# rrahn/libspm

Measured on AMD Instinct MI355X. Metric: Gbases/s scanned, Myers k<=3 |P|=100, higher is better.
Workload: dtype u32

## Files before the change

### libspm_amd/csrc/filter_dense.hpp

```cpp
#pragma once

#include "filter_stream.hpp"

namespace spm_hip
{

constexpr uint32_t kDenseQueueCap = 192;
constexpr int kDenseBatches = 3;

template <int NP>
__device__ __forceinline__ uint32_t dense_select(const filter_params &P, uint32_t w, uint32_t prev)
{
    const uint32_t X = alignbit(w, prev, 2);
    const uint32_t Y = alignbit(w, prev, 4);
    uint32_t sel = 0;
#pragma unroll
    for (int i = 0; i < NP; ++i) {
        const uint32_t C0 = (P.pat_c[i] & 3u) * 0x55555555u, M0 = (P.pat_cm[i] & 3u) * 0x55555555u;
        const uint32_t C1 = (P.pat_c[i] >> 2) * 0x55555555u, M1 = (P.pat_cm[i] >> 2) * 0x55555555u;
        uint32_t t = ((X ^ C0) & M0) | ((Y ^ C1) & M1);
        t |= t >> 1;
        sel |= ~t;
    }
    return sel & 0x55555555u;
// ... 38 lines not shown
            const uint32_t x0 = bk[b].x ^ f2, x1 = bk[b].y ^ f2, x2 = bk[b].z ^ f2, x3 = bk[b].w ^ f2;
            const uint32_t z = ((x0 - 0x00010001u) & ~x0) | ((x1 - 0x00010001u) & ~x1) | ((x2 - 0x00010001u) & ~x2) |
                               ((x3 - 0x00010001u) & ~x3);
            const bool hit = v[b] && ((z & 0x80008000u) != 0 || (bk[b].w >> 16) == kDenseAcceptAll);
            if (__ballot(hit) != 0) {
                if (__builtin_amdgcn_readfirstlane(cand_chunk_of(P, lds)[5]) == 0) {
                    const int64_t ts = (int64_t)span_base + (int64_t)off[b] - 16;
                    const bool has = hit && ts >= (int64_t)P.lo && (uint64_t)ts + P.key_len <= P.hi;
                    emit_survivors(P, has, key[b], has ? (uint64_t)ts : 0, lane, lds);
                }
            }
        }
    }
}

template <int UU, int NP, int S, bool KM>
__device__ __forceinline__ void dense_group(const filter_params &P, const uint4 (&cur)[UU], uint64_t gbase, uint64_t span_base,
                                            uint32_t &carry_in, uint32_t lane, const uint32_t *lds, dense_queue &Q, uint32_t &qn)
{
    static_assert(UU % 2 == 0 || UU == 1, "words are taken in pairs");
    uint32_t w[UU], prev[UU];
#pragma unroll
    for (int u = 0; u < UU; ++u)
        pack_with_prev(cur[u], lane, carry_in, w[u], prev[u]);
    const uint32_t goff = (uint32_t)(gbase - span_base) + lane * 16;
#pragma unroll
    for (int j = 0; j < UU; j += 2) {
        constexpr bool pair = UU > 1;
        const uint32_t w0 = w[j], p0 = prev[j], w1 = w[pair ? j + 1 : j], p1 = prev[pair ? j + 1 : j];
        const uint32_t kmask = KM ? P.key_mask : 0xFFFFFFFFu;
        static_assert(kDenseBloomBits == 20, "the word address below takes bits 5..19 of the index");
        uint32_t pm = 0;
        if constexpr (S == 0) {
            uint32_t todo = dense_select<NP>(P, w0, p0);
            if (pair)
                todo |= dense_select<NP>(P, w1, p1) << 1;
            while (todo != 0) {
                const uint32_t b = (uint32_t)__ffs(todo) - 1u;
                todo &= todo - 1;
                const bool odd = (b & 1u) != 0;
                const uint64_t both = ((uint64_t)(odd ? w1 : w0) << 32) | (odd ? p1 : p0);
                const uint32_t key = (uint32_t)(both >> ((b & ~1u) + 2u));
                const uint32_t h = key ^ (key >> 13);
                const uint32_t word = *reinterpret_cast<const uint32_t *>(reinterpret_cast<const uint8_t *>(lds) + ((h >> 3) & 0x1FFFCu));
                pm |= __builtin_amdgcn_ubfe(word, h, 1) << b;
            }
        } else {
#pragma unroll
            for (int u = 0; u < (pair ? 2 : 1); ++u) {
#pragma unroll
                for (int d = S; d <= 16; d += S) {
                    const uint32_t wu = u ? w1 : w0, pu = u ? p1 : p0;
                    const uint32_t key = (d == 16 ? wu : alignbit(wu, pu, (2 * d) & 31)) & kmask;
                    const uint32_t h = key ^ (key >> 13);
                    const uint32_t word = *reinterpret_cast<const uint32_t *>(reinterpret_cast<const uint8_t *>(lds) + ((h >> 3) & 0x1FFFCu));
                    pm |= __builtin_amdgcn_ubfe(word, h, 1) << (2 * (d - 1) + u);
                }
            }
        }
        while (__ballot(pm != 0) != 0) {
            const bool pos = pm != 0;
            const uint32_t b = pos ? (uint32_t)__ffs(pm) - 1u : 0u;
            pm &= pm - 1;
            const bool odd = (b & 1u) != 0;
            const uint64_t both = ((uint64_t)(odd ? w1 : w0) << 32) | (odd ? p1 : p0);
            const uint32_t key = (uint32_t)(both >> ((b & ~1u) + 2u)) & kmask;
            const uint64_t mm = __ballot(pos);
            if (pos) {
                const uint32_t q = qn + __popcll(mm & ((1ull << lane) - 1));
                Q.key[q] = key;
                Q.off[q] = goff + (uint32_t)j * 1024u + (odd ? 1024u : 0u) + (b >> 1) + 1u;
            }
            qn += __popcll(mm);
            queue_sync();
            if (qn > kDenseQueueCap - 64)
                dense_drain(P, Q, qn, false, span_base, lane, lds);
        }
    }
}

template <int U, int NP, int S = 0, bool KM = false>
__global__ __launch_bounds__(1024) void seed_filter_dense_kernel(const filter_params P)
{
    extern __shared__ uint32_t lds[];
    stream_stage(P, lds);

    const uint32_t lane = threadIdx.x & 63;
    const uint32_t waves_per_wg = blockDim.x >> 6;
    const uint32_t wave_in_wg = (uint32_t)__builtin_amdgcn_readfirstlane(threadIdx.x >> 6);
    dense_queue &Q = *reinterpret_cast<dense_queue *>(lds + P.lds_words + kCandLdsSlot + kCandRec * 16 +
                                                      (sizeof(dense_queue) / 4) * wave_in_wg);
    uint32_t qn = 0;

    const stream_geometry G = stream_geometry_of(P.lo, P.hi, 1024, P.span_chunks);
    const uint64_t span = P.span_chunks;
    const uint8_t *lane_text = P.text + G.base0 + (uint64_t)lane * 16;

    uint64_t sp;
    for (;;) {
        const span_draw drawn = draw_span(P, lds, lane, wave_in_wg, waves_per_wg, G.n_spans, sp);
        if (drawn == span_draw::done)
            break;
        if (drawn == span_draw::idle)
            continue;
        const uint64_t c_begin = sp * span;
        const uint64_t c_end = c_begin + span < G.n_chunks ? c_begin + span : G.n_chunks;
        const uint64_t span_base = G.base0 + c_begin * 1024;
        span_open(P, lds, lane, span_base);
        uint32_t carry_in = span_carry_in(P, span_base, lane);
        uint64_t ch = c_begin;
        const uint64_t whole_end = c_end < G.n_whole ? c_end : G.n_whole;
        const uint64_t fast_end = c_begin + (whole_end > c_begin ? (whole_end - c_begin) / U * U : 0);
        if (ch < fast_end) {
            uint4 nxt[U];
#pragma unroll
            for (int u = 0; u < U; ++u)
                nxt[u] = load16_stream(lane_text + (ch + u) * 1024);
            for (; ch < fast_end; ch += U) {
                uint4 cur[U];
#pragma unroll
                for (int u = 0; u < U; ++u)
                    cur[u] = nxt[u];
                const bool more = ch + U < fast_end;
                const uint64_t pf = more ? ch + U : ch;
                const uint64_t ustride = more ? 1024 : 0;
#pragma unroll
                for (int u = 0; u < U; ++u)
                    nxt[u] = load16_stream(lane_text + pf * 1024 + (uint64_t)u * ustride);
                __builtin_amdgcn_sched_barrier(0);
                dense_group<U, NP, S, KM>(P, cur, G.base0 + ch * 1024, span_base, carry_in, lane, lds, Q, qn);
            }
        }
        for (; ch < c_end; ++ch) {
            uint4 one[1];
            one[0] = load_text16(P.text, G.base0 + ch * 1024 + (uint64_t)lane * 16, P.hi);
            dense_group<1, NP, S, KM>(P, one, G.base0 + ch * 1024, span_base, carry_in, lane, lds, Q, qn);
        }
        dense_drain(P, Q, qn, true, span_base, lane, lds);
    }
    surv_close(P, cand_chunk_of(P, lds), lane);
}

}
```

### libspm_amd/csrc/filter_resolve.hpp

```cpp
#pragma once

#include "filter_params.hpp"
#include "pack.hpp"
#include "wave.hpp"

namespace spm_hip
{


__device__ __forceinline__ uint4 load_bytes16(const uint8_t *p)
{
    uint4 v;
    __builtin_memcpy(&v, p, 16);
    return v;
}

__device__ __forceinline__ uint4 load_bytes16_guarded(const uint8_t *base, uint64_t idx, uint64_t limit)
{
    if (idx + 16 <= limit)
        return load_bytes16(base + idx);
    uint32_t w[4] = {0xFFFFFFFFu, 0xFFFFFFFFu, 0xFFFFFFFFu, 0xFFFFFFFFu};
    for (int b = 0; b < 16; ++b)
        if (idx + b < limit)
            w[b >> 2] = (w[b >> 2] & ~(0xFFu << (8 * (b & 3)))) | ((uint32_t)base[idx + b] << (8 * (b & 3)));
// ... 306 lines not shown
        return;
    }
    if (live && through) {
        ++S.n_cand;
        d_hi = (int64_t)t - (int64_t)(val & 0x7FF) - sb + (int64_t)R.max_m;
        d_lo = d_hi - (int64_t)((rng & kRngRun) ? (rng & 0x7FF) : 0u);
        b_cur = d_lo / (int64_t)R.Bw;
        b_last = d_hi / (int64_t)R.Bw;
        if (R.overlap && b_cur > 0 && d_lo - b_cur * (int64_t)R.Bw <= (int64_t)R.k[pat])
            --b_cur;
        if ((uint64_t)b_last >> R.band_bits) {
            atomicAdd(&R.counters[kCntVoid], 1ull);
            b_last = b_cur - 1;
        }
    }
    for (;;) {
        const bool have = b_cur <= b_last;
        const uint64_t mm = __ballot(have);
        if (mm == 0)
            break;
        if (have) {
            const unsigned long long bkey =
                ((unsigned long long)pat << 43) | ((unsigned long long)seg << R.band_bits) | (unsigned long long)b_cur;
            const int64_t b0 = b_cur * (int64_t)R.Bw;
            const uint32_t o_lo = (uint32_t)(d_lo > b0 ? d_lo - b0 : 0);
            const uint32_t o_hi = (uint32_t)(d_hi < b0 + (int64_t)R.Bw - 1 ? d_hi - b0 : (int64_t)R.Bw - 1);
            const unsigned long long run = (o_hi - o_lo >= 63 ? ~0ull : ((1ull << (o_hi - o_lo + 1)) - 1)) << o_lo;
            const uint32_t q = S.bn + __popcll(mm & ((1ull << lane) - 1));
            B.key_lo[q] = (uint32_t)bkey;
            B.key_hi[q] = (uint32_t)(bkey >> 32);
            B.run_lo[q] = (uint32_t)run;
            B.run_hi[q] = (uint32_t)(run >> 32);
        }
        S.bn += __popcll(mm);
        queue_sync();
        if (S.bn >= 64) {
            S.bn -= 64;
            insert_bands(R, B, S.bn, 64, lane, S.C);
            queue_sync();
        }
        ++b_cur;
    }
    queue_sync();
}

__global__ __launch_bounds__(256) void resolve_kernel(const resolve_params R)
{
    __shared__ pair_queue pair_queues[4];
    __shared__ band_queue band_queues[4];
    unsigned long long n = R.counters[kCntSurvSlots];
    if (blockIdx.x == 0 && threadIdx.x == 0) {
        atomicAdd(&R.counters[kCntUnreadSurvSum], n);
        atomicMax(&R.counters[kCntUnreadSurvMax], n);
    }
    if (n > R.surv_cap)
        n = R.surv_cap;
    if (!R.exact_hits && __hip_atomic_load(R.table_poison, __ATOMIC_RELAXED, __HIP_MEMORY_SCOPE_AGENT) != 0) {
        if (blockIdx.x == 0 && threadIdx.x == 0)
            atomicAdd(&R.counters[kCntVoid], 1ull);
        return;
    }
    const uint32_t lane = threadIdx.x & 63;
    resolve_wave S;
    S.Q = &pair_queues[threadIdx.x >> 6];
    S.B = &band_queues[threadIdx.x >> 6];
    S.qn = 0;
    S.bn = 0;
    S.C.base = 0;
    S.C.used = 0;
    S.C.size = 0;
    S.C.draws = 0;
    S.n_cand = 0;
    pair_queue &Q = *S.Q;
    const uint64_t stride = (uint64_t)gridDim.x * blockDim.x;
    const uint64_t rounds = (n + stride - 1) / stride;
    for (uint64_t r = 0; r < rounds; ++r) {
        if ((r & 7u) == 7u &&
            __builtin_amdgcn_readfirstlane((uint32_t)(__hip_atomic_load(&R.counters[kCntVoid], __ATOMIC_RELAXED, __HIP_MEMORY_SCOPE_AGENT) != 0)))
            break;
        const uint64_t i = r * stride + (uint64_t)blockIdx.x * blockDim.x + threadIdx.x;
        bool probing = false;
        uint32_t key = 0;
        uint64_t t = 0, seg = 0;
        pass_entry T = R.passes[0];
        if (i < n) {
            const survivor sv = R.surv[i];
            if (sv.t_hi != kSurvInvalid) {
                probing = true;
                key = sv.key;
                t = ((uint64_t)sv.t_hi << 32) | sv.t_lo;
                if (sv.pad != 0)
                    T = R.passes[sv.pad];
            }
        }
        if (probing && R.seg_offsets) {
            uint64_t lo = 0, hi = R.n_segments;
            while (hi - lo > 1) {
                const uint64_t mid = (lo + hi) >> 1;
                if (R.seg_offsets[mid] <= t)
                    lo = mid;
                else
                    hi = mid;
            }
            seg = lo;
            if ((int64_t)t + (int64_t)R.key_len > (int64_t)R.seg_offsets[lo + 1])
                probing = false;
        }
        text64 W;
        W.lo = 0;
        W.hi = 0;
        W.ok = false;
        if (probing && R.flank_check) {
            int64_t sb = (int64_t)R.hay_begin, se = (int64_t)R.hay_end;
            if (R.seg_offsets) {
                sb = (int64_t)R.seg_offsets[seg];
                se = (int64_t)R.seg_offsets[seg + 1];
            }
            if ((int64_t)t - 16 >= sb && (int64_t)t + 48 <= se && t + 48 <= R.text_alloc) {
                const uint8_t *p = R.text + (t - 16);
                W.lo = (uint64_t)pack16(load_bytes16(p)) | ((uint64_t)pack16(load_bytes16(p + 16)) << 32);
                W.hi = (uint64_t)pack16(load_bytes16(p + 32)) | ((uint64_t)pack16(load_bytes16(p + 48)) << 32);
                W.ok = true;
            }
        }
        uint32_t first = 0, cnt = 0;
        {
            uint32_t slot = ht_hash(key) & T.ht_mask;
            while (__ballot(probing) != 0) {
                if (probing) {
                    const uint4 d = T.ht[slot];
                    if (d.z == 0) {
                        probing = false;
                    } else if (d.x == key) {
                        first = d.y;
                        cnt = d.z;
                        probing = false;
                    } else {
                        slot = (slot + 1) & T.ht_mask;
                    }
                }
            }
        }
        uint32_t incl = cnt;
#pragma unroll
        for (int o = 1; o < 64; o <<= 1) {
            const uint32_t up = (uint32_t)__shfl_up((int)incl, o);
            if (lane >= (uint32_t)o)
                incl += up;
        }
        const uint32_t total = (uint32_t)__builtin_amdgcn_readfirstlane(__shfl((int)incl, 63));
        for (uint32_t p0 = 0; p0 < total; p0 += 64) {
            const uint32_t i = p0 + lane;
            bool have = i < total;
            uint32_t owner = 0;
#pragma unroll
            for (int step = 32; step > 0; step >>= 1) {
                const uint32_t v = (uint32_t)__shfl((int)incl, (int)(owner + step - 1));
                if (v <= i)
                    owner += step;
            }
            owner = owner > 63 ? 63 : owner;
            const uint32_t o_incl = (uint32_t)__shfl((int)incl, (int)owner), o_cnt = (uint32_t)__shfl((int)cnt, (int)owner);
            const uint32_t o_first = (uint32_t)__shfl((int)first, (int)owner);
            const uint64_t o_t = ((uint64_t)(uint32_t)__shfl((int)(uint32_t)(t >> 32), (int)owner) << 32) |
                                 (uint32_t)__shfl((int)(uint32_t)t, (int)owner);
            const uint32_t o_seg = (uint32_t)__shfl((int)(uint32_t)seg, (int)owner);
            text64 OW;
            OW.lo = ((uint64_t)(uint32_t)__shfl((int)(uint32_t)(W.lo >> 32), (int)owner) << 32) |
                    (uint32_t)__shfl((int)(uint32_t)W.lo, (int)owner);
            OW.hi = ((uint64_t)(uint32_t)__shfl((int)(uint32_t)(W.hi >> 32), (int)owner) << 32) |
                    (uint32_t)__shfl((int)(uint32_t)W.hi, (int)owner);
            OW.ok = __shfl((int)W.ok, (int)owner) != 0;
            uint32_t val = 0, rng = 0;
            if (have) {
                const uint4 e = R.entries[o_first + (i - (o_incl - o_cnt))];
                val = e.x;
                rng = e.z;
                if (!(rng & kRngRun)) {
                    const uint32_t r0 = rng & 0x1F, ns = (rng >> 5) & 0x1F;
                    const bool whole = (rng & kRngWhole) != 0;
                    rng = (r0 << 16) | (whole ? (ns << 5) | kRngWhole : 0u);
                    if (OW.ok) {
                        if (!seed_sig_ok(OW, e.y, r0, ns, R.key_len))
                            have = false;
                        else if (whole)
                            rng |= kSeedChecked;
                    }
                }
            }
            const uint64_t mm = __ballot(have);
            if (mm != 0) {
                if (have) {
                    const uint32_t q = S.qn + __popcll(mm & ((1ull << lane) - 1));
                    Q.t_lo[q] = (uint32_t)o_t;
                    Q.t_hi[q] = (uint32_t)(o_t >> 32);
                    Q.val[q] = val;
                    Q.rng[q] = rng;
                    Q.seg[q] = o_seg;
                }
                S.qn += __popcll(mm);
                queue_sync();
                while (S.qn >= 64)
                    check_pairs(R, S, 64, lane);
            }
        }
    }
    while (S.qn != 0)
        check_pairs(R, S, S.qn < 64 ? S.qn : 64, lane);
    if (S.bn != 0)
        insert_bands(R, *S.B, 0, S.bn, lane, S.C);
    for (uint32_t q = S.C.used + lane; q < S.C.size; q += 64)
        if (S.C.base + q < R.band_cap)
            R.bands[S.C.base + q].val = kBandInvalid;
    wave_count_add(R.counters + kCntPairs, S.n_cand);
}

}
```

### libspm_amd/csrc/filter_stream.hip

```cpp
#include "filter_launch.hpp"
#include "filter_stream.hpp"

namespace
{
using packed_kernel = void (*)(filter_params, const uint4 *);

template <int S, int U, bool KM>
filter_kernel sparse_kernel(uint32_t hv, uint32_t sigma)
{
    if (hv == 2 && sigma == 5)
        return seed_filter_kernel<S, U, 2, 5, KM>;
    if (hv == 2 && sigma == 15)
        return seed_filter_kernel<S, U, 2, 15, KM>;
    if (hv == 1 && sigma == 4)
        return seed_filter_kernel<S, U, 1, 4, KM>;
    if constexpr (S >= 4)
        if (hv == 2 && sigma == 4)
            return seed_filter_kernel<S, U, 2, 4, KM>;
    return nullptr;
}

filter_kernel select_filter_kernel(const filter_index &F, uint32_t sigma, bool km)
{
    if (F.dense || F.hash_variant == 4)
        return select_dense_kernel(F, km);
    switch (F.stride) {
    case 16: return km ? nullptr : sparse_kernel<16, 8, false>(F.hash_variant, sigma);
    case 8: return km ? nullptr : sparse_kernel<8, 8, false>(F.hash_variant, sigma);
    case 4: return km ? nullptr : sparse_kernel<4, 8, false>(F.hash_variant, sigma);
    case 2: return km ? sparse_kernel<2, 2, true>(F.hash_variant, sigma) : sparse_kernel<2, 2, false>(F.hash_variant, sigma);
    case 1:
        if (F.anchor_cm != 0 && F.hash_variant == 2 && sigma == 4 && !km)
            return seed_filter_kernel<1, 4, 2, 4, false, true>;
        return km ? sparse_kernel<1, 2, true>(F.hash_variant, sigma) : sparse_kernel<1, 2, false>(F.hash_variant, sigma);
    default: return nullptr;
    }
}

packed_kernel select_packed_kernel(uint32_t stride, bool km)
{
    if (km)
        return nullptr;
    switch (stride) {
    case 16: return seed_filter_packed_kernel<16, 4, 2, false>;
    case 8: return seed_filter_packed_kernel<8, 4, 2, false>;
    case 4: return seed_filter_packed_kernel<4, 2, 2, false>;
    default: return nullptr;
    }
}

}

int launch_stream_pass(const scan_args &A, filter_params P, uint32_t pass)
{
    spm_ctx *ctx = A.ctx;
    const spm_patterns *ps = A.ps;
    spm_hits *H = A.hits;
    const filter_index &F = ps->fidx[pass];
    P.stride = F.stride;
    P.key_len = F.key_len;
    P.key_mask = F.key_len >= 16 ? 0xFFFFFFFFu : ((1u << (2 * F.key_len)) - 1);
    P.bitmap_words = F.hash_variant == 2 ? 1024 : F.bitmap_words;
    P.lds_words = F.lds_words;
    P.chd_slot_mask = F.chd_slot_mask;
    P.chd_bucket_shift = F.chd_bucket_shift;
    P.chd_disp_off = F.chd_disp_off;
    P.n_probes = F.n_probes;
    P.bitmap = F.d_bitmap;
    P.pass = pass;
    P.anchor_c = F.anchor_c;
    P.anchor_cm = F.anchor_cm;
    P.n_pat = F.n_pat;
    for (uint32_t i = 0; i < kDensePatterns; ++i) {
        P.pat_c[i] = F.pat_c[i];
        P.pat_cm[i] = F.pat_cm[i];
    }
    P.bucket_shift = F.bucket_shift;
    P.buckets = reinterpret_cast<const uint4 *>(F.d_buckets);
    const bool km = F.key_len < 16;
    const bool bits = F.hash_variant == 4;
    const bool use_packed = F.hash_variant == 2 && A.text->d_packed && ps->sigma == 4 && F.stride >= 2 &&
                            !(A.opts.flags & SPM_SCAN_IGNORE_PACKED);
    const bool wide_ok = use_packed || F.stride == 2 || (F.stride == 1 && !km && ps->sigma == 4);
    const uint32_t threads = (F.dense || bits || wide_ok) ? 1024 : 512;
    const size_t lds = (size_t)F.lds_words * 4 + 16 + 16 * kCandRec * 4 + ((F.dense || bits) ? 16 * kDenseQueueBytes : 0);
    const uint32_t wg_per_cu = (uint32_t)std::max<size_t>(1, std::min<size_t>((160 * 1024) / lds, 2048 / threads));
    const uint32_t grid = ctx->n_cu * wg_per_cu;
    const uint64_t n_waves = (uint64_t)grid * (threads / 64);
    const span_plan span = plan_span(stream_geometry_of(P.lo, P.hi, 1024).n_chunks, n_waves, 1024);
    P.span_chunks = span.span_chunks;
    P.span_unit = 1024;
    const int sb = A.tune.span_budget;
    P.span_budget = sb > 0 ? (uint32_t)sb : (uint32_t)std::max<uint64_t>(256, (uint64_t)span.span_chunks * 1024 / 4);
    P.dynamic = span.dynamic;
    P.hash_variant = F.hash_variant;
    H->stats.span_symbols = P.span_chunks * P.span_unit;
    if (use_packed) {
        filter_params Q = P;
        const span_plan pspan = plan_span(stream_geometry_of(Q.lo, Q.hi, 4096).n_chunks, n_waves, 4096);
        Q.span_chunks = pspan.span_chunks;
        Q.span_unit = 4096;
        if (sb <= 0)
            Q.span_budget = (uint32_t)std::max<uint64_t>(256, (uint64_t)pspan.span_chunks * 4096 / 4);
        Q.dynamic = pspan.dynamic;
        H->stats.span_symbols = Q.span_chunks * Q.span_unit;
        const packed_kernel k = select_packed_kernel(F.stride, km);
        if (!k) {
            SPM_SET_ERR(ctx, "internal: no packed filter kernel for stride %u, key length %u", F.stride, F.key_len);
            return SPM_E_UNSUPPORTED;
        }
        launch(k, dim3(grid), threads, lds, ctx->stream, Q, reinterpret_cast<const uint4 *>(A.text->d_packed));
    } else {
        const filter_kernel k = select_filter_kernel(F, ps->sigma, km);
        if (!k) {
            SPM_SET_ERR(ctx, "internal: no filter kernel for stride %u, key length %u, sigma %u, hash variant %u, %u patterns",
                        F.stride, F.key_len, ps->sigma, F.hash_variant, F.n_pat);
            return SPM_E_UNSUPPORTED;
        }
        launch(k, dim3(grid), threads, lds, ctx->stream, P);
    }
    return SPM_OK;
}

void warm_stream_kernels()
{
    hipFuncAttributes a;
    (void)hipFuncGetAttributes(&a, (const void *)seed_filter_kernel<16, 8, 2, 4, false>);
}
```

### libspm_amd/csrc/filter_stream.hpp

```cpp
#pragma once

#include "brute.hpp"
#include "filter_params.hpp"
#include "pack.hpp"

namespace spm_hip
{

__device__ __forceinline__ uint32_t *cand_chunk_of(const filter_params &P, const uint32_t *lds)
{
    const uint32_t wave = (uint32_t)__builtin_amdgcn_readfirstlane(threadIdx.x >> 6);
    return const_cast<uint32_t *>(lds) + P.lds_words + kCandLdsSlot + kCandRec * wave;
}

__device__ __forceinline__ void span_open(const filter_params &P, const uint32_t *lds, uint32_t lane, uint64_t begin)
{
    if (lane == 0) {
        uint32_t *ck = cand_chunk_of(P, lds);
        ck[4] = 0;
        ck[5] = 0;
        ck[6] = (uint32_t)begin;
        ck[7] = (uint32_t)(begin >> 32);
    }
}
// ... 168 lines not shown
    }
    while (__ballot(pos_mask != 0) != 0) {
        if (__builtin_amdgcn_readfirstlane(cand_chunk_of(P, lds)[5]) != 0)
            break;
        uint64_t t = 0;
        uint32_t key = 0;
        bool has = false;
        if (pos_mask != 0) {
            const int bit = __ffs(pos_mask) - 1;
            pos_mask &= pos_mask - 1;
            const int u = bit / NWIN, i = bit % NWIN;
            const int d = S * (i + 1);
            uint32_t wu = w[0], pu = prev[0];
#pragma unroll
            for (int q = 1; q < NWD; ++q)
                if (u == q) {
                    wu = w[q];
                    pu = prev[q];
                }
            key = (d == 16 ? wu : alignbit(wu, pu, (uint32_t)(2 * d) & 31u)) & kmask;
            const uint64_t wpos = PK ? gbase + (uint64_t)(u >> 2) * 4096 + (uint64_t)lane * 64 + (uint64_t)(u & 3) * 16
                                     : gbase + (uint64_t)u * 1024 + (uint64_t)lane * 16;
            const int64_t ts = (int64_t)wpos - 16 + d;
            if (ts >= (int64_t)P.lo && (uint64_t)ts + P.key_len <= P.hi) {
                t = (uint64_t)ts;
                has = true;
            }
        }
        emit_survivors(P, has, key, t, lane, lds);
    }
}



__device__ __forceinline__ uint32_t anchor_select(uint32_t w, uint32_t prev, uint32_t c, uint32_t cm)
{
    const uint32_t C0 = (c & 3u) * 0x55555555u, M0 = (cm & 3u) * 0x55555555u;
    const uint32_t C1 = (c >> 2) * 0x55555555u, M1 = (cm >> 2) * 0x55555555u;
    const uint32_t X = alignbit(w, prev, 2);
    const uint32_t Y = alignbit(w, prev, 4);
    uint32_t t = ((X ^ C0) & M0) | ((Y ^ C1) & M1);
    t |= t >> 1;
    return ~t & 0x55555555u;
}

template <int NWD>
__device__ __forceinline__ void filter_words_anchored(const filter_params &P, const uint32_t (&w)[NWD], const uint32_t (&prev)[NWD],
                                                      uint64_t gbase, uint32_t lane, const uint32_t *lds)
{
    static_assert(NWD % 2 == 0 || NWD == 1, "words are taken in pairs");
    const uint16_t *fp_tab = reinterpret_cast<const uint16_t *>(lds);
    const uint16_t *disp_tab = reinterpret_cast<const uint16_t *>(reinterpret_cast<const uint8_t *>(lds) + P.chd_disp_off);
#pragma unroll
    for (int j = 0; j < NWD; j += 2) {
        uint32_t todo = anchor_select(w[j], prev[j], P.anchor_c, P.anchor_cm);
        if (j + 1 < NWD)
            todo |= anchor_select(w[j + 1 < NWD ? j + 1 : j], prev[j + 1 < NWD ? j + 1 : j], P.anchor_c, P.anchor_cm) << 1;
        while (__ballot(todo != 0) != 0) {
            const bool act = todo != 0;
            const uint32_t b = act ? (uint32_t)__ffs(todo) - 1u : 0u;
            todo &= todo - 1;
            const uint32_t u = b & 1u, d = (b >> 1) + 1u;
            const uint32_t wu = (j + 1 < NWD && u) ? w[j + 1 < NWD ? j + 1 : j] : w[j];
            const uint32_t pu = (j + 1 < NWD && u) ? prev[j + 1 < NWD ? j + 1 : j] : prev[j];
            const uint32_t key = (uint32_t)((((uint64_t)wu << 32) | pu) >> (2 * d));
            const uint32_t x = chd_hash(key).x;
            const uint32_t dsp = disp_tab[x >> P.chd_bucket_shift];
            const uint32_t slot = ((x >> 3) + dsp * ((key | 1u) & 0xFFFFFFu)) & P.chd_slot_mask;
            const uint32_t f = fp_tab[slot];
            const bool hit = act && ((f ^ key ^ (key >> 16)) & 0xFFFFu) == 0;
            if (__ballot(hit) != 0) {
                if (__builtin_amdgcn_readfirstlane(cand_chunk_of(P, lds)[5]) != 0)
                    return;
                const uint64_t wpos = gbase + (uint64_t)(j + u) * 1024 + (uint64_t)lane * 16;
                const int64_t ts = (int64_t)wpos - 16 + (int64_t)d;
                const bool has = hit && ts >= (int64_t)P.lo && (uint64_t)ts + P.key_len <= P.hi;
                emit_survivors(P, has, key, has ? (uint64_t)ts : 0, lane, lds);
            }
        }
    }
}


__device__ __forceinline__ void stream_stage(const filter_params &P, uint32_t *lds)
{
    for (uint32_t i = threadIdx.x; i < P.lds_words; i += blockDim.x)
        lds[i] = P.bitmap[i];
    if ((threadIdx.x & 63) == 0) {
        uint32_t *ck = lds + P.lds_words + kCandLdsSlot + kCandRec * (threadIdx.x >> 6);
        for (uint32_t i = 0; i < kCandRec; ++i)
            ck[i] = 0;
    }
    __syncthreads();
}

enum class span_draw
{
    run,
    idle,
    done,
};

__device__ __forceinline__ span_draw draw_span(const filter_params &P, uint32_t *lds, uint32_t lane, uint32_t wave_in_wg,
                                               uint32_t waves_per_wg, uint64_t n_spans, uint64_t &sp)
{
    if (P.dynamic == 1) {
        unsigned long long t = 0;
        if (lane == 0)
            t = atomicAdd(&P.counters[kCntSpanHead], 1ull);
        sp = uniform_u64(t);
        return sp >= n_spans ? span_draw::done : span_draw::run;
    }
    __syncthreads();
    if (threadIdx.x == 0) {
        const unsigned long long t = atomicAdd(&P.counters[kCntSpanHead], (unsigned long long)waves_per_wg);
        lds[P.lds_words] = (uint32_t)t;
        lds[P.lds_words + 1] = (uint32_t)(t >> 32);
    }
    __syncthreads();
    const uint64_t base = uniform_u64(((uint64_t)lds[P.lds_words + 1] << 32) | lds[P.lds_words]);
    if (base >= n_spans)
        return span_draw::done;
    sp = base + wave_in_wg;
    return sp >= n_spans ? span_draw::idle : span_draw::run;
}

template <int SIG>
__device__ __forceinline__ uint32_t span_carry_in(const filter_params &P, uint64_t span_base, uint32_t lane, uint32_t &carry_n)
{
    uint32_t carry_in = 0;
    carry_n = 0;
    if (span_base >= 16 && lane == 0) {
        const uint4 before = load_text16(P.text, span_base - 16, P.hi);
        carry_in = pack16_sig<SIG>(before, carry_n);
    }
    carry_n = __builtin_amdgcn_readfirstlane(carry_n);
    return __builtin_amdgcn_readfirstlane(carry_in);
}

__device__ __forceinline__ uint32_t span_carry_in(const filter_params &P, uint64_t span_base, uint32_t lane)
{
    uint32_t no_n;
    return span_carry_in<4>(P, span_base, lane, no_n);
}

__device__ __forceinline__ void pack_with_prev(const uint4 &cur, uint32_t lane, uint32_t &carry_in, uint32_t &w, uint32_t &prev)
{
    w = pack16(cur);
    prev = __builtin_amdgcn_update_dpp(0u, w, 0x138 , 0xF, 0xF, false);
    if (lane == 0)
        prev = carry_in;
    carry_in = __builtin_amdgcn_readlane(w, 63);
}

template <int S, int UU, int HV, int SIG, bool KM, bool AN = false>
__device__ __forceinline__ void filter_group(const filter_params &P, const uint4 (&cur)[UU], uint64_t gbase,
                                             uint32_t &carry_in, uint32_t &carry_n, uint32_t lane,
                                             const uint32_t *lds, uint32_t idx_mask)
{
    uint32_t w[UU], prev[UU];
    uint32_t nv[SIG != 4 ? UU : 1];
#pragma unroll
    for (int u = 0; u < UU; ++u) {
        if constexpr (SIG == 4) {
            pack_with_prev(cur[u], lane, carry_in, w[u], prev[u]);
        } else {
            uint32_t nm = 0;
            w[u] = pack16_sig<SIG>(cur[u], nm);
            prev[u] = __builtin_amdgcn_update_dpp(0u, w[u], 0x138 , 0xF, 0xF, false);
            if (lane == 0)
                prev[u] = carry_in;
            carry_in = __builtin_amdgcn_readlane(w[u], 63);
            uint32_t np = __builtin_amdgcn_update_dpp(0u, nm, 0x138, 0xF, 0xF, false);
            if (lane == 0)
                np = carry_n;
            carry_n = __builtin_amdgcn_readlane(nm, 63);
            nv[u] = (nm << 16) | np;
        }
    }
    if constexpr (AN)
        filter_words_anchored<UU>(P, w, prev, gbase, lane, lds);
    else
        filter_words<S, UU, HV, SIG, false, KM>(P, w, prev, nv, gbase, lane, lds, idx_mask);
}

template <int S, int U, int HV, int SIG, bool KM, bool AN = false>
__global__ __launch_bounds__(((S == 1 && !KM && SIG == 4) || (S == 2 && U == 2)) ? 1024 : 512) void seed_filter_kernel(const filter_params P)
{
    extern __shared__ uint32_t lds[];
    stream_stage(P, lds);

    const uint32_t lane = threadIdx.x & 63;
    const uint32_t waves_per_wg = blockDim.x >> 6;
    const uint32_t wave_in_wg = (uint32_t)__builtin_amdgcn_readfirstlane(threadIdx.x >> 6);
    const uint32_t idx_mask = P.bitmap_words * 32 - 1;

    const stream_geometry G = stream_geometry_of(P.lo, P.hi, 1024, P.span_chunks);
    const uint64_t span = P.span_chunks;
    const uint8_t *lane_text = P.text + G.base0 + (uint64_t)lane * 16;

    uint64_t sp;
    for (;;) {
        const span_draw drawn = draw_span(P, lds, lane, wave_in_wg, waves_per_wg, G.n_spans, sp);
        if (drawn == span_draw::done)
            break;
        if (drawn == span_draw::idle)
            continue;
        const uint64_t c_begin = sp * span;
        const uint64_t c_end = c_begin + span < G.n_chunks ? c_begin + span : G.n_chunks;
        span_open(P, lds, lane, G.base0 + c_begin * 1024);
        uint32_t carry_n;
        uint32_t carry_in = span_carry_in<SIG>(P, G.base0 + c_begin * 1024, lane, carry_n);
        uint64_t ch = c_begin;
        const uint64_t whole_end = c_end < G.n_whole ? c_end : G.n_whole;
        const uint64_t fast_end = c_begin + (whole_end > c_begin ? (whole_end - c_begin) / U * U : 0);
        if (ch < fast_end) {
            uint4 nxt[U];
#pragma unroll
            for (int u = 0; u < U; ++u)
                nxt[u] = load16_stream(lane_text + (ch + u) * 1024);
            for (; ch < fast_end; ch += U) {
                uint4 cur[U];
#pragma unroll
                for (int u = 0; u < U; ++u)
                    cur[u] = nxt[u];
                const bool more = ch + U < fast_end;
                const uint64_t pf = more ? ch + U : ch;
                const uint64_t ustride = more ? 1024 : 0;
#pragma unroll
                for (int u = 0; u < U; ++u)
                    nxt[u] = load16_stream(lane_text + pf * 1024 + (uint64_t)u * ustride);
                if constexpr (S <= 2)
                    __builtin_amdgcn_sched_barrier(0);
                filter_group<S, U, HV, SIG, KM, AN>(P, cur, G.base0 + ch * 1024, carry_in, carry_n, lane, lds, idx_mask);
            }
        }
        for (; ch < c_end; ++ch) {
            uint4 one[1];
            one[0] = load_text16(P.text, (G.base0 + ch * 1024) | ((uint64_t)lane * 16), P.hi);
            filter_group<S, 1, HV, SIG, KM, AN>(P, one, G.base0 + ch * 1024, carry_in, carry_n, lane, lds, idx_mask);
        }
    }
    surv_close(P, cand_chunk_of(P, lds), lane);
}

template <int S, int U2, int HV, bool KM>
__global__ __launch_bounds__(1024) void seed_filter_packed_kernel(const filter_params P, const uint4 *__restrict__ shadow)
{
    extern __shared__ uint32_t lds[];
    stream_stage(P, lds);

    constexpr int NWD = 4 * U2;
    const uint32_t lane = threadIdx.x & 63;
    const uint32_t waves_per_wg = blockDim.x >> 6;
    const uint32_t wave_in_wg = (uint32_t)__builtin_amdgcn_readfirstlane(threadIdx.x >> 6);
    const uint32_t idx_mask = P.bitmap_words * 32 - 1;

    const stream_geometry G = stream_geometry_of(P.lo, P.hi, 4096, P.span_chunks);
    const uint64_t span = P.span_chunks;
    const uint4 *lane_src = shadow + (G.base0 / 64) + lane;

    uint64_t sp;
    for (;;) {
        const span_draw drawn = draw_span(P, lds, lane, wave_in_wg, waves_per_wg, G.n_spans, sp);
        if (drawn == span_draw::done)
            break;
        if (drawn == span_draw::idle)
            continue;
        const uint64_t c_begin = sp * span;
        const uint64_t c_end = c_begin + span < G.n_chunks ? c_begin + span : G.n_chunks;
        const uint64_t fast_end = c_begin + (c_end - c_begin + U2 - 1) / U2 * U2;
        span_open(P, lds, lane, G.base0 + c_begin * 4096);
        uint32_t carry_in = 0;
        {
            const uint64_t first_word = (G.base0 + c_begin * 4096) / 16;
            if (first_word > 0 && lane == 0)
                carry_in = reinterpret_cast<const uint32_t *>(shadow)[first_word - 1];
            carry_in = __builtin_amdgcn_readfirstlane(carry_in);
        }
        uint4 nxt[U2];
#pragma unroll
        for (int u = 0; u < U2; ++u)
            nxt[u] = load16_stream(reinterpret_cast<const uint8_t *>(lane_src + (c_begin + u) * 64));
        for (uint64_t ch = c_begin; ch < fast_end; ch += U2) {
            uint4 cur[U2];
#pragma unroll
            for (int u = 0; u < U2; ++u)
                cur[u] = nxt[u];
            const bool more = ch + U2 < fast_end;
            const uint64_t pf = more ? ch + U2 : ch;
            const uint64_t ustride = more ? 64 : 0;
#pragma unroll
            for (int u = 0; u < U2; ++u)
                nxt[u] = load16_stream(reinterpret_cast<const uint8_t *>(lane_src + pf * 64 + (uint64_t)u * ustride));
            __builtin_amdgcn_sched_barrier(0);
            uint32_t w[NWD], prev[NWD];
            const uint32_t nv[1] = {0};
#pragma unroll
            for (int u = 0; u < U2; ++u) {
                w[4 * u + 0] = cur[u].x;
                w[4 * u + 1] = cur[u].y;
                w[4 * u + 2] = cur[u].z;
                w[4 * u + 3] = cur[u].w;
                uint32_t p0 = __builtin_amdgcn_update_dpp(0u, cur[u].w, 0x138 , 0xF, 0xF, false);
                if (lane == 0)
                    p0 = carry_in;
                carry_in = __builtin_amdgcn_readlane(cur[u].w, 63);
                prev[4 * u + 0] = p0;
                prev[4 * u + 1] = cur[u].x;
                prev[4 * u + 2] = cur[u].y;
                prev[4 * u + 3] = cur[u].z;
            }
            filter_words<S, NWD, HV, 4, true, KM>(P, w, prev, nv, G.base0 + ch * 4096, lane, lds, idx_mask);
        }
    }
    surv_close(P, cand_chunk_of(P, lds), lane);
}

}
```

### libspm_amd/csrc/filter_verify.hpp

```cpp
#pragma once

#include "brute.hpp"
#include "filter_params.hpp"
#include "pack.hpp"
#include "wave.hpp"

namespace spm_hip
{

__device__ __forceinline__ bool seen_insert(const verify_params &P, uint32_t pat, int64_t e)
{
    return seen_insert_raw(P.seen, P.seen_mask, P.overflow, pat, e);
}

__global__ __launch_bounds__(256) void band_select_kernel(const verify_params P, band_rec *out, unsigned long long *out_count)
{
    unsigned long long n = P.counters[kCntBandSlots];
    if (n > P.band_cap)
        n = P.band_cap;
    const uint32_t lane = threadIdx.x & 63;
    const uint64_t stride = (uint64_t)gridDim.x * blockDim.x;
    const uint64_t rounds = (n + stride - 1) / stride;
    for (uint64_t r = 0; r < rounds; ++r) {
        const uint64_t i = r * stride + (uint64_t)blockIdx.x * blockDim.x + threadIdx.x;
// ... 89 lines not shown
            }
            c.val = (c.val & ~0x7FFu) | code;
            mine[j] = c;
        }
        uint32_t c01 = 0, c23 = 0;
#pragma unroll
        for (uint32_t j = 0; j < PER; ++j)
            if (head_mask & (1u << j)) {
                const uint32_t cls = (mine[j].val >> kRunLenShift) & kRunLenMask;
                const uint32_t one = 1u << (16 * (cls & 1u));
                c01 += cls < 2 ? one : 0u;
                c23 += cls < 2 ? 0u : one;
            }
        uint32_t i01 = c01, i23 = c23;
#pragma unroll
        for (int o = 1; o < 64; o <<= 1) {
            const uint32_t u01 = (uint32_t)__shfl_up((int)i01, o), u23 = (uint32_t)__shfl_up((int)i23, o);
            if (lane >= (uint32_t)o) {
                i01 += u01;
                i23 += u23;
            }
        }
        if (lane == 63) {
            wave_tot01[wave] = i01;
            wave_tot23[wave] = i23;
        }
        __syncthreads();
        uint32_t off01 = 0, off23 = 0, tot01 = 0, tot23 = 0;
        for (uint32_t w = 0; w < 4; ++w) {
            off01 += w < wave ? wave_tot01[w] : 0u;
            off23 += w < wave ? wave_tot23[w] : 0u;
            tot01 += wave_tot01[w];
            tot23 += wave_tot23[w];
        }
        const uint32_t tot[4] = {tot01 & 0xFFFFu, tot01 >> 16, tot23 & 0xFFFFu, tot23 >> 16};
        const uint32_t total = tot[0] + tot[1] + tot[2] + tot[3];
        if (tid == 0)
            chunk_base = total ? atomicAdd(head_count, (unsigned long long)total) : 0ull;
        __syncthreads();
        const uint32_t mine_before[4] = {(off01 & 0xFFFFu) + ((i01 - c01) & 0xFFFFu), (off01 >> 16) + ((i01 - c01) >> 16),
                                         (off23 & 0xFFFFu) + ((i23 - c23) & 0xFFFFu), (off23 >> 16) + ((i23 - c23) >> 16)};
        uint64_t pos[4];
        pos[0] = chunk_base + mine_before[0];
        pos[1] = chunk_base + tot[0] + mine_before[1];
        pos[2] = chunk_base + tot[0] + tot[1] + mine_before[2];
        pos[3] = chunk_base + tot[0] + tot[1] + tot[2] + mine_before[3];
#pragma unroll
        for (uint32_t j = 0; j < PER; ++j)
            if (head_mask & (1u << j)) {
                const uint32_t cls = (mine[j].val >> kRunLenShift) & kRunLenMask;
                const uint64_t at = cls == 0 ? pos[0] : cls == 1 ? pos[1] : cls == 2 ? pos[2] : pos[3];
                heads[at] = mine[j];
                pos[0] += cls == 0 ? 1u : 0u;
                pos[1] += cls == 1 ? 1u : 0u;
                pos[2] += cls == 2 ? 1u : 0u;
                pos[3] += cls == 3 ? 1u : 0u;
            }
        __syncthreads();
    }
}

__global__ __launch_bounds__(256) void band_release_kernel(const verify_params P, const band_rec *bands, uint32_t counter)
{
    unsigned long long n = P.counters[counter];
    if (n > P.band_cap)
        n = P.band_cap;
    const uint64_t stride = (uint64_t)gridDim.x * blockDim.x;
    for (uint64_t i = (uint64_t)blockIdx.x * blockDim.x + threadIdx.x; i < n; i += stride) {
        const band_rec c = bands[i];
        if (c.val != kBandInvalid)
            band_release(P.band_tab, c.slot);
    }
}

struct band_geom
{
    uint32_t pat;
    int64_t m, k;
    int64_t e_lo, e_hi;
    int64_t ws;
    int64_t dd_lo, dd_hi;
};

__device__ __forceinline__ bool decode_band(const verify_params &P, const band_rec &c, bool consume, band_geom &g)
{
    if (c.val == kBandInvalid)
        return false;
    g.pat = c.val >> 11;
    unsigned long long v = 1;
    if (!P.preselected) {
        v = band_value(P.band_tab[c.slot].y, P.overlap != 0);
        if (consume)
            band_release(P.band_tab, c.slot);
        if (c.val & kRunFollower)
            return false;
        if (P.overlap ? (uint32_t)v < (P.surplus ? (uint32_t)P.surplus[g.pat] : 1u) : v == 0)
            return false;
    }
    g.m = P.m[g.pat];
    g.k = P.k[g.pat];
    int64_t own_b = (int64_t)P.scan_begin, own_e = (int64_t)P.scan_end, hay_b = (int64_t)P.ctx_begin;
    if (P.seg_offsets) {
        const int64_t sb = (int64_t)P.seg_offsets[c.seg], se = (int64_t)P.seg_offsets[c.seg + 1];
        own_b = P.seg_owned ? sb + (int64_t)P.seg_owned[c.seg] : sb;
        own_e = se;
        hay_b = sb;
    }
    const int64_t band_base = hay_b - (int64_t)P.max_m + (int64_t)c.band * (int64_t)P.Bw;
    int64_t d = band_base;
    int64_t span = (int64_t)P.Bw - 1 + (P.overlap ? g.k + 1 : 0);
    if (!P.overlap) {
        const int lo = __ffsll((long long)v) - 1;
        int hi = 63 - __clzll((long long)v);
        if (c.val & kRunAnalysed)
            hi = (int)(((c.val >> kRunLenShift) & kRunLenMask) * P.Bw + (c.val & kRunHiMask));
        d += lo;
        span = hi - lo;
    }
    g.e_lo = d + g.m - g.k;
    g.e_hi = d + g.m + g.k + span;
    g.dd_lo = INT64_MAX;
    g.dd_hi = INT64_MIN;
    if (!P.overlap && (c.val & kRunAnalysed) && !P.seg_offsets) {
        const int64_t next_base = band_base + (int64_t)(((c.val >> kRunLenShift) & kRunLenMask) + 1) * (int64_t)P.Bw;
        g.dd_lo = (c.val & kRunTouchLeft) ? band_base + g.m + g.k : INT64_MIN;
        g.dd_hi = (c.val & kRunTouchRight) ? next_base + g.m - g.k - 1 : INT64_MAX;
    }
    if (g.e_lo < own_b + 1)
        g.e_lo = own_b + 1;
    if (g.e_hi > own_e)
        g.e_hi = own_e;
    if (g.e_lo > g.e_hi)
        return false;
    g.ws = g.e_lo - (g.m + g.k);
    if (g.ws < hay_b)
        g.ws = hay_b;
    return true;
}

template <int NWN>
__global__ __launch_bounds__(256) void verify_kernel(const verify_params P)
{
    extern __shared__ uint32_t vlds[];
    const uint32_t tid = threadIdx.x;
    const uint32_t nthr = blockDim.x;
    const uint32_t rows = P.sigma + 1;
    uint16_t *hitbuf = reinterpret_cast<uint16_t *>(vlds + (size_t)rows * NWN * nthr);
    spm_hit *stage = reinterpret_cast<spm_hit *>(hitbuf + (size_t)16 * nthr) + (size_t)(tid >> 6) * kHitStage;
    uint32_t n_staged = 0;
    const uint32_t lane = tid & 63;
    auto flush = [&]() {
        if (n_staged == 0)
            return;
        unsigned long long base = 0;
        if (lane == 0)
            base = atomicAdd(P.hit_counter, (unsigned long long)n_staged);
        base = uniform_u64(base);
        for (uint32_t i = lane; i < n_staged; i += 64)
            if (base + i < P.hit_cap)
                P.hits[base + i] = stage[i];
        n_staged = 0;
        queue_sync();
    };
    unsigned long long n_cand = P.counters[P.band_counter];
    if (n_cand > P.band_cap)
        n_cand = P.band_cap;
    const uint64_t stride = (uint64_t)gridDim.x * nthr;
    uint32_t n_valid = 0;
    const uint64_t rounds = (n_cand + stride - 1) / stride;
    for (uint64_t rd = 0; rd < rounds; ++rd) {
        const uint64_t ci = rd * stride + (uint64_t)blockIdx.x * nthr + tid;
        band_geom g;
        g.pat = 0;
        g.m = 1;
        g.k = 0;
        g.e_lo = 0;
        g.e_hi = -1;
        g.ws = 0;
        const bool active = ci < n_cand && decode_band(P, P.bands[ci], P.runs == 0, g);
        if (active)
            ++n_valid;
        const uint32_t pat = g.pat;
        const int64_t m = g.m, k = g.k, e_lo = g.e_lo, e_hi = active ? g.e_hi : g.ws, ws = g.ws;
        const uint32_t *src = P.peq32 + (((size_t)(pat >> 6) * rows) * P.nw_table + (P.nw_table - NWN)) * 64 + (pat & 63);
        if (active)
            for (uint32_t r = 0; r < rows; ++r)
#pragma unroll
                for (int w = 0; w < NWN; ++w)
                    vlds[((size_t)r * NWN + w) * nthr + tid] = src[((size_t)r * P.nw_table + w) * 64];
        myers_lane<NWN, false> L;
        {
            const int32_t off = NWN * 32 - (int32_t)m;
#pragma unroll
            for (int w = 0; w < NWN; ++w) {
                const int32_t lo = off - w * 32;
                L.VP[w] = lo <= 0 ? 0xFFFFFFFFu : (lo >= 32 ? 0u : (0xFFFFFFFFu << lo));
                L.VN[w] = 0;
            }
            L.score = (int32_t)m;
        }
        const int64_t blk0 = ws & ~15ll;
        uint4 nxt = make_uint4(0, 0, 0, 0);
        if (active)
            nxt = load_text16(P.text, (uint64_t)blk0, P.text_alloc);
        const uint32_t n_cols = (uint32_t)(e_hi - ws);
        const uint32_t rel_lo = (uint32_t)(e_lo - 1 - ws);
        const uint32_t sigma = P.sigma;
        uint32_t rel0 = (uint32_t)(blk0 - ws);
        const uint32_t my_blocks = active ? (uint32_t)((e_hi - blk0 + 15) >> 4) : 0u;
        uint32_t max_blocks = my_blocks;
        for (int o = 32; o > 0; o >>= 1)
            max_blocks = max(max_blocks, (uint32_t)__shfl_xor((int)max_blocks, o));
        max_blocks = (uint32_t)__builtin_amdgcn_readfirstlane(max_blocks);
        for (uint32_t bi = 0; bi < max_blocks; ++bi, rel0 += 16) {
            const int64_t blk = blk0 + 16 * (int64_t)bi;
            uint32_t hitmask = 0;
            if (bi < my_blocks) {
                const uint4 cur = nxt;
                if (bi + 1 < my_blocks)
                    nxt = load_text16(P.text, (uint64_t)(blk + 16), P.text_alloc);
                const uint32_t words[4] = {cur.x, cur.y, cur.z, cur.w};
#pragma unroll
                for (int i = 0; i < 16; ++i) {
                    const uint32_t rel = rel0 + (uint32_t)i;
                    if (rel >= n_cols)
                        continue;
                    uint32_t sym = (words[i >> 2] >> (8 * (i & 3))) & 0xFF;
                    sym = sym < sigma ? sym : sigma;
                    L.step_strided(vlds + ((size_t)sym * NWN) * nthr + tid, nthr);
                    if (L.score <= (int32_t)k && rel >= rel_lo) {
                        hitbuf[(size_t)i * nthr + tid] = (uint16_t)(L.score + 1);
                        hitmask |= 1u << i;
                    }
                }
            }
            if (__ballot(hitmask != 0) == 0)
                continue;
            uint32_t fresh = 0, keep = 0;
            for (uint32_t mm = hitmask; mm != 0; mm &= mm - 1) {
                const uint32_t i = (uint32_t)__ffs(mm) - 1u;
                const int64_t e = blk + (int64_t)i + 1;
                if ((e > g.dd_lo && e < g.dd_hi) || seen_insert(P, pat, e)) {
                    ++fresh;
                    keep |= 1u << i;
                }
            }
            uint32_t incl = fresh;
#pragma unroll
            for (int o = 1; o < 64; o <<= 1) {
                const uint32_t up = (uint32_t)__shfl_up((int)incl, o);
                if (lane >= (uint32_t)o)
                    incl += up;
            }
            const uint32_t total = (uint32_t)__builtin_amdgcn_readfirstlane(__shfl((int)incl, 63));
            if (total == 0)
                continue;
            if (n_staged + total > kHitStage)
                flush();
            unsigned long long direct = 0;
            const bool staged = total <= kHitStage;
            if (!staged) {
                if (lane == 0)
                    direct = atomicAdd(P.hit_counter, (unsigned long long)total);
                direct = uniform_u64(direct);
            }
            uint32_t at = n_staged + incl - fresh;
            for (uint32_t mm = keep; mm != 0; mm &= mm - 1) {
                const uint32_t i = (uint32_t)__ffs(mm) - 1u;
                const int64_t e = blk + (int64_t)i + 1;
                spm_hit h;
                h.pos = (P.report_begin ? (uint64_t)(e - m) : (uint64_t)e) + P.pos_offset;
                h.pattern = pat;
// ... 243 lines not shown
```

Before: 6515.

## Batch global loads for memory-level parallelism across filter, resolve and verify kernels

```diff
diff --git a/libspm_amd/csrc/filter_dense.hpp b/libspm_amd/csrc/filter_dense.hpp
--- a/libspm_amd/csrc/filter_dense.hpp
+++ b/libspm_amd/csrc/filter_dense.hpp
@@ -144,8 +144,8 @@
 template <int U, int NP, int S = 0, bool KM = false>
 __global__ __launch_bounds__(1024) void seed_filter_dense_kernel(const filter_params P)
 {
-    extern __shared__ uint32_t lds[];
-    stream_stage(P, lds);
+    extern __shared__ __align__(16) uint32_t lds[];
+    stream_stage<8>(P, lds);
 
     const uint32_t lane = threadIdx.x & 63;
     const uint32_t waves_per_wg = blockDim.x >> 6;
diff --git a/libspm_amd/csrc/filter_resolve.hpp b/libspm_amd/csrc/filter_resolve.hpp
--- a/libspm_amd/csrc/filter_resolve.hpp
+++ b/libspm_amd/csrc/filter_resolve.hpp
@@ -412,16 +412,15 @@
         bool probing = false;
         uint32_t key = 0;
         uint64_t t = 0, seg = 0;
+        uint4 raw = *reinterpret_cast<const uint4 *>(R.surv + (i < n ? i : n - 1));
         pass_entry T = R.passes[0];
-        if (i < n) {
-            const survivor sv = R.surv[i];
-            if (sv.t_hi != kSurvInvalid) {
-                probing = true;
-                key = sv.key;
-                t = ((uint64_t)sv.t_hi << 32) | sv.t_lo;
-                if (sv.pad != 0)
-                    T = R.passes[sv.pad];
-            }
+        asm volatile("" : "+v"(raw.x), "+v"(raw.y), "+v"(raw.z), "+v"(raw.w));
+        if (i < n && raw.z != kSurvInvalid) {
+            probing = true;
+            key = raw.x;
+            t = ((uint64_t)raw.z << 32) | raw.y;
+            if (raw.w != 0)
+                T = R.passes[raw.w];
         }
         if (probing && R.seg_offsets) {
             uint64_t lo = 0, hi = R.n_segments;
@@ -436,6 +435,8 @@
             if ((int64_t)t + (int64_t)R.key_len > (int64_t)R.seg_offsets[lo + 1])
                 probing = false;
         }
+        uint32_t slot = ht_hash(key) & T.ht_mask;
+        uint4 d = T.ht[slot];
         text64 W;
         W.lo = 0;
         W.hi = 0;
@@ -448,17 +449,19 @@
             }
             if ((int64_t)t - 16 >= sb && (int64_t)t + 48 <= se && t + 48 <= R.text_alloc) {
                 const uint8_t *p = R.text + (t - 16);
-                W.lo = (uint64_t)pack16(load_bytes16(p)) | ((uint64_t)pack16(load_bytes16(p + 16)) << 32);
-                W.hi = (uint64_t)pack16(load_bytes16(p + 32)) | ((uint64_t)pack16(load_bytes16(p + 48)) << 32);
+                uint4 tb[4];
+#pragma unroll
+                for (int j = 0; j < 4; ++j)
+                    tb[j] = load_bytes16(p + 16 * j);
+                W.lo = (uint64_t)pack16(tb[0]) | ((uint64_t)pack16(tb[1]) << 32);
+                W.hi = (uint64_t)pack16(tb[2]) | ((uint64_t)pack16(tb[3]) << 32);
                 W.ok = true;
             }
         }
         uint32_t first = 0, cnt = 0;
         {
-            uint32_t slot = ht_hash(key) & T.ht_mask;
             while (__ballot(probing) != 0) {
                 if (probing) {
-                    const uint4 d = T.ht[slot];
                     if (d.z == 0) {
                         probing = false;
                     } else if (d.x == key) {
@@ -467,6 +470,7 @@
                         probing = false;
                     } else {
                         slot = (slot + 1) & T.ht_mask;
+                        d = T.ht[slot];
                     }
                 }
             }
diff --git a/libspm_amd/csrc/filter_stream.hip b/libspm_amd/csrc/filter_stream.hip
--- a/libspm_amd/csrc/filter_stream.hip
+++ b/libspm_amd/csrc/filter_stream.hip
@@ -67,6 +67,10 @@
     P.chd_disp_off = F.chd_disp_off;
     P.n_probes = F.n_probes;
     P.bitmap = F.d_bitmap;
+    if (reinterpret_cast<uintptr_t>(P.bitmap) % 16 != 0) {
+        SPM_SET_ERR(ctx, "internal: the level-1 image of pass %u is not 16-byte aligned", pass);
+        return SPM_E_UNSUPPORTED;
+    }
     P.pass = pass;
     P.anchor_c = F.anchor_c;
     P.anchor_cm = F.anchor_cm;
diff --git a/libspm_amd/csrc/filter_stream.hpp b/libspm_amd/csrc/filter_stream.hpp
--- a/libspm_amd/csrc/filter_stream.hpp
+++ b/libspm_amd/csrc/filter_stream.hpp
@@ -274,9 +274,26 @@
 }
 
 
+template <int DEPTH>
 __device__ __forceinline__ void stream_stage(const filter_params &P, uint32_t *lds)
 {
-    for (uint32_t i = threadIdx.x; i < P.lds_words; i += blockDim.x)
+    const uint32_t n4 = P.lds_words >> 2;
+    const uint4 *src = reinterpret_cast<const uint4 *>(P.bitmap);
+    uint4 *dst = reinterpret_cast<uint4 *>(lds);
+    for (uint32_t base = 0; base < n4; base += DEPTH * blockDim.x) {
+        uint4 v[DEPTH];
+        uint32_t at[DEPTH];
+#pragma unroll
+        for (int j = 0; j < DEPTH; ++j) {
+            const uint32_t i = base + j * blockDim.x + threadIdx.x;
+            at[j] = i < n4 ? i : n4 - 1;
+            v[j] = src[at[j]];
+        }
+#pragma unroll
+        for (int j = 0; j < DEPTH; ++j)
+            dst[at[j]] = v[j];
+    }
+    for (uint32_t i = 4 * n4 + threadIdx.x; i < P.lds_words; i += blockDim.x)
         lds[i] = P.bitmap[i];
     if ((threadIdx.x & 63) == 0) {
         uint32_t *ck = lds + P.lds_words + kCandLdsSlot + kCandRec * (threadIdx.x >> 6);
@@ -379,8 +396,8 @@
 template <int S, int U, int HV, int SIG, bool KM, bool AN = false>
 __global__ __launch_bounds__(((S == 1 && !KM && SIG == 4) || (S == 2 && U == 2)) ? 1024 : 512) void seed_filter_kernel(const filter_params P)
 {
-    extern __shared__ uint32_t lds[];
-    stream_stage(P, lds);
+    extern __shared__ __align__(16) uint32_t lds[];
+    stream_stage<((S == 1 && !KM && SIG == 4) || (S == 2 && U == 2)) ? 9 : 18>(P, lds);
 
     const uint32_t lane = threadIdx.x & 63;
     const uint32_t waves_per_wg = blockDim.x >> 6;
@@ -439,8 +456,8 @@
 template <int S, int U2, int HV, bool KM>
 __global__ __launch_bounds__(1024) void seed_filter_packed_kernel(const filter_params P, const uint4 *__restrict__ shadow)
 {
-    extern __shared__ uint32_t lds[];
-    stream_stage(P, lds);
+    extern __shared__ __align__(16) uint32_t lds[];
+    stream_stage<9>(P, lds);
 
     constexpr int NWD = 4 * U2;
     const uint32_t lane = threadIdx.x & 63;
diff --git a/libspm_amd/csrc/filter_verify.hpp b/libspm_amd/csrc/filter_verify.hpp
--- a/libspm_amd/csrc/filter_verify.hpp
+++ b/libspm_amd/csrc/filter_verify.hpp
@@ -195,14 +195,15 @@
     int64_t dd_lo, dd_hi;
 };
 
-__device__ __forceinline__ bool decode_band(const verify_params &P, const band_rec &c, bool consume, band_geom &g)
+__device__ __forceinline__ bool decode_band(const verify_params &P, const band_rec &c, bool consume, band_geom &g, int32_t m, int32_t k,
+                                            unsigned long long stored)
 {
     if (c.val == kBandInvalid)
         return false;
     g.pat = c.val >> 11;
     unsigned long long v = 1;
     if (!P.preselected) {
-        v = band_value(P.band_tab[c.slot].y, P.overlap != 0);
+        v = band_value(stored, P.overlap != 0);
         if (consume)
             band_release(P.band_tab, c.slot);
         if (c.val & kRunFollower)
@@ -210,8 +211,8 @@
         if (P.overlap ? (uint32_t)v < (P.surplus ? (uint32_t)P.surplus[g.pat] : 1u) : v == 0)
             return false;
     }
-    g.m = P.m[g.pat];
-    g.k = P.k[g.pat];
+    g.m = m;
+    g.k = k;
     int64_t own_b = (int64_t)P.scan_begin, own_e = (int64_t)P.scan_end, hay_b = (int64_t)P.ctx_begin;
     if (P.seg_offsets) {
         const int64_t sb = (int64_t)P.seg_offsets[c.seg], se = (int64_t)P.seg_offsets[c.seg + 1];
@@ -249,6 +250,14 @@
     if (g.ws < hay_b)
         g.ws = hay_b;
     return true;
+}
+
+__device__ __forceinline__ bool decode_band(const verify_params &P, const band_rec &c, bool consume, band_geom &g)
+{
+    if (c.val == kBandInvalid)
+        return false;
+    const unsigned long long stored = P.preselected ? 0ull : P.band_tab[c.slot].y;
+    return decode_band(P, c, consume, g, P.m[c.val >> 11], P.k[c.val >> 11], stored);
 }
 
 template <int NWN>
@@ -290,17 +299,45 @@
         g.e_lo = 0;
         g.e_hi = -1;
         g.ws = 0;
-        const bool active = ci < n_cand && decode_band(P, P.bands[ci], P.runs == 0, g);
+        band_rec c;
+        c.slot = c.seg = c.band = 0;
+        c.val = kBandInvalid;
+        if (ci < n_cand)
+            c = P.bands[ci];
+        const bool listed = c.val != kBandInvalid;
+        int32_t m_pat = 1, k_pat = 0;
+        unsigned long long stored = 0;
+        if (listed) {
+            const uint32_t p = c.val >> 11;
+            if (!P.preselected)
+                stored = P.band_tab[c.slot].y;
+            m_pat = P.m[p];
+            k_pat = P.k[p];
+            const uint32_t *src = P.peq32 + (((size_t)(p >> 6) * rows) * P.nw_table + (P.nw_table - NWN)) * 64 + (p & 63);
+            constexpr int RB = NWN <= 4 ? 8 : NWN <= 8 ? 4 : NWN <= 16 ? 2 : 1;
+            for (uint32_t r0 = 0; r0 < rows; r0 += RB) {
+                uint32_t v[RB][NWN];
+#pragma unroll
+                for (int j = 0; j < RB; ++j) {
+                    const uint32_t r = r0 + j < rows ? r0 + j : rows - 1;
+#pragma unroll
+                    for (int w = 0; w < NWN; ++w)
+                        v[j][w] = src[((size_t)r * P.nw_table + w) * 64];
+                }
+#pragma unroll
+                for (int j = 0; j < RB; ++j) {
+                    const uint32_t r = r0 + j < rows ? r0 + j : rows - 1;
+#pragma unroll
+                    for (int w = 0; w < NWN; ++w)
+                        vlds[((size_t)r * NWN + w) * nthr + tid] = v[j][w];
+                }
+            }
+        }
+        const bool active = decode_band(P, c, P.runs == 0, g, m_pat, k_pat, stored);
         if (active)
             ++n_valid;
         const uint32_t pat = g.pat;
         const int64_t m = g.m, k = g.k, e_lo = g.e_lo, e_hi = active ? g.e_hi : g.ws, ws = g.ws;
-        const uint32_t *src = P.peq32 + (((size_t)(pat >> 6) * rows) * P.nw_table + (P.nw_table - NWN)) * 64 + (pat & 63);
-        if (active)
-            for (uint32_t r = 0; r < rows; ++r)
-#pragma unroll
-                for (int w = 0; w < NWN; ++w)
-                    vlds[((size_t)r * NWN + w) * nthr + tid] = src[((size_t)r * P.nw_table + w) * 64];
         myers_lane<NWN, false> L;
         {
             const int32_t off = NWN * 32 - (int32_t)m;
```

Measured after the change: 6528 (median of 6 runs). No clear change (+0.2%).
